# zdwww/EgoGaussian

Measured on AMD Instinct MI355X. Metric: train iters/s (fwd+bwd render) + PSNR, 500k Gaussians @ 960x540, higher is better.
Workload: dtype f32

## Files before the change

egogaussian_amd/csrc/api.hip:

```cpp
#include "egs_common.h"
#include "object_motion.h"
#include "backward_prologue.h"
#include "loss_window.h"
#include "label_bce.h"
#include "opacity_entropy.h"
#include <string.h>
#include <vector>
#include <mutex>
#include <unordered_map>
#include <stdlib.h>

namespace {

struct GeomLayout { egs_geom_layout o; size_t bytes; };
struct BinLayout { egs_binning_layout o; size_t bytes; };
struct ImgLayout { egs_image_layout o; size_t bytes; };

GeomLayout geom_layout(int P) {
    GeomLayout L; size_t off = 0; const size_t n = (size_t)(P > 0 ? P : 0);
    L.o.rec = off;          off = egs_align(off + n * sizeof(float4) * EGS_SPLAT_REC_F4);
    L.o.rect = off;         off = egs_align(off + n * sizeof(uint2));
    L.o.offsets = off;      off = egs_align(off + n * sizeof(uint32_t));
    L.o.clamped = off;      off = egs_align(off + n);
    L.o.visible = off;      off = egs_align(off + n);
// ... 498 lines not shown
        if (!entropy->weight || !entropy->n_vis || (P > 0 && !entropy->scratch) || c.obj_loss) return EGS_ERR_ARG;
        if (sc.act & EGS_ACT_OBJECT_MOTION) return EGS_ERR_MODE;
    }
    EgsObjRot orot; MotionHost mh; rc = obj_motion_args(sc, c.rot, orot, mh); if (rc) return rc;
    EgsLossGradHost lgh = {}; const EgsLossGradHost* lgp = nullptr; EgsObjLossK olk = {};
    if (c.obj_loss && !c.loss_grad) return EGS_ERR_ARG;
    if (c.loss_grad) {
        const egs_loss_grad& q = *c.loss_grad;
        if (!q.image || !q.gt || !q.dm_dmu1 || !q.dm_dexx || !q.dm_dexy || !q.upstream_grad) return EGS_ERR_ARG;
        if (c.dL_dout_depth || c.dL_dout_alpha || (c.grad_mask == EGS_GRAD_COLORS && sc.colors && !sink && !st.grad_accum)) return EGS_ERR_MODE;
        lgh = EgsLossGradHost{ q.image, q.gt, q.dm_dmu1, q.dm_dexx, q.dm_dexy, q.gate, q.upstream_grad, nullptr, 1.f - q.lambda_dssim, q.lambda_dssim,
                               q.deferred_partial_sums, q.deferred_partial_sums ? egs_l1_ssim_partial_count(3, height, width) / 2 : 0, q.lambda_dssim,
                               q.deferred_loss, q.deferred_partial_sums ? q.loss_running_sum : nullptr };
        lgp = &lgh;
        if (!dL_dout_color) dL_dout_color = q.image;
        if (c.obj_loss) {
            if (q.deferred_partial_sums && !c.obj_loss->alpha_partial_sums) return EGS_ERR_ARG;
            rc = obj_loss_args(c.obj_loss, 3, height, width, q.lambda_dssim, olk); if (rc) return rc;
            lgh.w_l1_n = c.obj_loss->lambda_image * (1.f - q.lambda_dssim); lgh.w_ssim_n = c.obj_loss->lambda_image * q.lambda_dssim;
            lgh.obj = &olk;
        }
    }
    if (P == 0) {
        if (lgp) EGS_TRY(egs_launch_loss_finish(lgh, width, height, s));
        if (entropy) EGS_TRY(egs_launch_entropy_reduce(0, nullptr, nullptr, 0, nullptr, nullptr, nullptr, nullptr, entropy->n_vis, entropy->value, s));
        if (mh.grad) EGS_TRY(egs_launch_zero_u32((uint32_t*)mh.grad, EGS_MOTION_SUMS, s));
        return 0;
    }
    if (R < 0 || R >= (1ll << 31)) return EGS_ERR_RANGE;
    if (c.grad_mask & ~EGS_GRAD_MASK_BITS) return EGS_ERR_ARG;
    const bool colors_only = c.grad_mask == EGS_GRAD_COLORS && sc.colors && !sink && !st.grad_accum;
    if (!c.background || lacks_pointers(sc, cam, c.radii, c.geom_buffer) || !c.image_buffer || !dL_dout_color || (!d.means2D && !colors_only) || !c.scratch)
        return EGS_ERR_ARG;
    if (misaligned(c.geom_buffer, c.binning_buffer, c.image_buffer) || ((uintptr_t)c.scratch & 15u)) return EGS_ERR_ARG;
    EgsGeomPtrs g = geom_ptrs(const_cast<void*>(c.geom_buffer), P);
    float* grad_acc = (float*)c.scratch;
    if (colors_only) {
        if (entropy) return EGS_ERR_MODE;
        if (!d.colors || (R > 0 && !c.binning_buffer)) return EGS_ERR_ARG;
        rc = check_modes(sc); if (rc) return rc;
        if (R == 0) return (int)egs_launch_zero_u32((uint32_t*)d.colors, (size_t)P * 3, s);
        EgsBinPtrs b = bin_ptrs(const_cast<void*>(c.binning_buffer), P, R, width, height);
        EgsImgPtrs im = img_ptrs(const_cast<void*>(c.image_buffer), width, height);
        if (!c.prologue_done) EGS_TRY(egs_launch_backward_prologue(P, width, height, im, grad_acc, g.block_hot, nullptr, s));
        void* det = nullptr; rc = det_lines_clear(c.scratch, P, debug, s, &det); if (rc) return rc;
        egs_prof_start(EGS_K_RENDER_BWD, s);
        EGS_TRY(egs_launch_render_backward(P, width, height, c.background, g, b.point_list, im, dL_dout_color, nullptr, nullptr, grad_acc, 1, nullptr, s, det));
        egs_prof_stop(EGS_K_RENDER_BWD, s);
        EGS_SYNC_IF_DEBUG(s);
        egs_prof_start(EGS_K_PREPROCESS_BWD, s);
        EGS_TRY(egs_launch_colors_from_acc(P, grad_acc, g.clamped, c.radii, d.colors, s));
        if (mh.grad) EGS_TRY(egs_launch_zero_u32((uint32_t*)mh.grad, EGS_MOTION_SUMS, s));
        egs_prof_stop(EGS_K_PREPROCESS_BWD, s);
        EGS_SYNC_IF_DEBUG(s);
        return 0;
    }
    const bool sh_apart = egs_sh_apart(sc);
    bool own[EGS_SINK_LEAVES] = { false, false, false, false, false, false };
    const bool sh_sink_ok = sh_apart && egs_sh_backward_can_sink(sc.M, sc.shs, sc.shs_rest);
    if (sink) {
        if (!sink->coef) return EGS_ERR_ARG;
        for (int l = 0; l < EGS_SINK_LEAVES; l++) {
            const egs_adam_leaf& f = sink->leaf[l];
            own[l] = f.param != nullptr;
            if (own[l] && (!f.exp_avg || !f.exp_avg_sq || !f.lr || !f.step)) return EGS_ERR_ARG;
        }
        if ((own[EGS_SINK_SCALES] || own[EGS_SINK_ROTATIONS]) && sc.cov3D) return EGS_ERR_MODE;
// ... 92 lines not shown
    return backward_impl({ BWD_SCENE, dL_dout_color, dL_dout_depth, dL_dout_alpha, BWD_OUTPUTS, BWD_SINK_TAIL, nullptr, nullptr, nullptr });
}

int egs_backward_lossgrad(int P, int sh_degree, int sh_coeffs, int64_t R, const float* background, const float* means3D,
                          const float* shs, const float* shs_rest, const float* colors_precomp, const float* scales, float scale_modifier,
                          const float* rotations, const float* cov3D_precomp, int activation_flags, const float* viewmatrix, const float* projmatrix,
                          const float* campos, int width, int height, float tan_fovx, float tan_fovy, const int32_t* radii,
                          const void* geom_buffer, const void* binning_buffer, const void* image_buffer, const egs_loss_grad* loss_grad,
                          float* dL_dmeans2D, float* dL_dcolors, float* dL_dopacity, float* dL_dmeans3D, float* dL_dcov3D, float* dL_dsh, float* dL_dsh_rest,
                          float* dL_dscales, float* dL_drotations, float* stat_grad_accum, float* stat_denom, float* stat_max_radii,
                          const uint32_t* skip_flag, const egs_adam_sink* sink, int prologue_done, const egs_object_rotation* rot, int grad_mask, void* scratch,
                          void* stream, int debug) {
    if (!loss_grad) return EGS_ERR_ARG;
    return backward_impl({ BWD_SCENE, nullptr, nullptr, nullptr, BWD_OUTPUTS, BWD_SINK_TAIL, loss_grad, nullptr, nullptr });
}

int egs_backward_entropy_lossgrad(int P, int sh_degree, int sh_coeffs, int64_t R, const float* background, const float* means3D,
                          const float* shs, const float* shs_rest, const float* colors_precomp, const float* scales, float scale_modifier,
                          const float* rotations, const float* cov3D_precomp, int activation_flags, const float* viewmatrix, const float* projmatrix,
                          const float* campos, int width, int height, float tan_fovx, float tan_fovy, const int32_t* radii,
                          const void* geom_buffer, const void* binning_buffer, const void* image_buffer, const egs_loss_grad* loss_grad,
                          const egs_opacity_entropy* entropy, const float* dL_dout_color, const float* dL_dout_depth, const float* dL_dout_alpha,
                          float* dL_dmeans2D, float* dL_dcolors, float* dL_dopacity, float* dL_dmeans3D, float* dL_dcov3D, float* dL_dsh, float* dL_dsh_rest,
                          float* dL_dscales, float* dL_drotations, float* stat_grad_accum, float* stat_denom, float* stat_max_radii,
                          const uint32_t* skip_flag, const egs_adam_sink* sink, int prologue_done, const egs_object_rotation* rot, int grad_mask, void* scratch,
                          void* stream, int debug) {
    if (!entropy) return EGS_ERR_ARG;
    if (loss_grad && (dL_dout_color || dL_dout_depth || dL_dout_alpha)) return EGS_ERR_MODE;
    return backward_impl({ BWD_SCENE, dL_dout_color, dL_dout_depth, dL_dout_alpha, BWD_OUTPUTS, BWD_SINK_TAIL, loss_grad, nullptr, entropy });
}

static int prologue_args(const egs_backward_prologue* side, EgsPrologueArgs& pa) {
    int rc = check_dims(side->P, side->width, side->height); if (rc) return rc;
    if (side->P <= 0 || !side->image_buffer || !side->scratch) return EGS_ERR_ARG;
    EgsImgPtrs im = img_ptrs(side->image_buffer, side->width, side->height);
    pa.n_tiles = (int)egs_tiles(side->width, side->height);
    pa.quad_work = im.quad_work; pa.tile_order = im.tile_order;
    if (side->geom_buffer && misaligned(side->geom_buffer)) return EGS_ERR_ARG;
    egs_prologue_acc(pa, (float*)side->scratch, (size_t)side->P,
                     side->geom_buffer ? geom_ptrs(const_cast<void*>(side->geom_buffer), side->P).block_hot : nullptr);
    if (side->sink) {
        if (!side->sink->coef) return EGS_ERR_ARG;
        EgsSink ks = {};
        sink_to_kernel_args(side->sink, side->skip_flag, ks, pa.tick);
        pa.has_tick = 1;
    }
    return 0;
}

int egs_l1_ssim_backward_ex(int channels, int height, int width, const float* img, const float* gt, float lambda_dssim,
                            const float* upstream_grad, const float* gate, const float* dm_dmu1, const float* dm_dexx,
                            const float* dm_dexy, float* dL_dimg, const float* deferred_partial_sums, float* deferred_loss,
                            float* loss_running_sum, const egs_backward_prologue* side, void* stream) {
    if (!side)
        return egs_launch_l1_ssim_backward(channels, height, width, img, gt, lambda_dssim, upstream_grad, gate, dm_dmu1, dm_dexx, dm_dexy, dL_dimg,
                                           deferred_partial_sums, deferred_loss, loss_running_sum, nullptr, (hipStream_t)stream);
    EgsPrologueArgs pa = {};
    int rc = prologue_args(side, pa); if (rc) return rc;
    return egs_launch_l1_ssim_backward(channels, height, width, img, gt, lambda_dssim, upstream_grad, gate, dm_dmu1, dm_dexx, dm_dexy, dL_dimg,
                                       deferred_partial_sums, deferred_loss, loss_running_sum, &pa, (hipStream_t)stream);
}

int egs_l1_ssim_forward_ex(int channels, int height, int width, const float* img, const float* gt, float lambda_dssim,
                           float* partial_sums, float* dm_dmu1, float* dm_dexx, float* dm_dexy, float* loss, float* loss_running_sum,
                           const egs_backward_prologue* side, void* stream) {
    EgsPrologueArgs pa = {};
    if (side) { int rc = prologue_args(side, pa); if (rc) return rc; }
// ... 62 lines not shown
}
int egs_label_bce_backward(int height, int width, const float* img, const float* obj_mask, const float* gate, const float* upstream_grad, float* dL_dimg,
                           const float* deferred_partial_sums, float* deferred_loss, float* loss_running_sum, void* stream) {
    int rc = check_dims(0, width, height); if (rc) return rc;
    if (!img || !obj_mask || !upstream_grad || !dL_dimg) return EGS_ERR_ARG;
    EGS_TRY(egs_launch_label_bce_backward(height, width, img, obj_mask, gate, upstream_grad, dL_dimg, deferred_partial_sums, deferred_loss,
                                          deferred_partial_sums ? loss_running_sum : nullptr, (hipStream_t)stream));
    return 0;
}
int egs_backward_label(int P, int64_t R, int width, int height, const int32_t* radii, const void* geom_buffer, const void* binning_buffer,
                       const void* image_buffer, const float* dL_dout_color, const egs_label_loss* loss, float* dL_dlabel, const egs_adam_leaf* adam,
                       float beta1, float beta2, float eps, float* coef, const int32_t* active_rows, const uint32_t* skip_flag, void* scratch,
                       void* stream, int flags) {
    const int debug = flags;
    int rc = check_dims(P, width, height); if (rc) return rc;
    if ((dL_dout_color != nullptr) == (loss != nullptr)) return EGS_ERR_MODE;
    if (R < 0 || R >= (1ll << 31)) return EGS_ERR_RANGE;
    const size_t n_partial = egs_label_bce_partial_count(height, width);
    if (loss && (!loss->img || !loss->mask || !loss->upstream || !loss->partial || loss->n_partial < n_partial)) return EGS_ERR_ARG;
    if (adam && (!adam->param || !adam->exp_avg || !adam->exp_avg_sq || !adam->lr || !adam->step || !coef)) return EGS_ERR_ARG;
    hipStream_t s = (hipStream_t)stream;
    const float inv_hw = 1.f / ((float)height * (float)width);
    EgsAdamTick tick = {}; EgsLabelAdam la = {};
    if (adam) {
        tick.step[0] = adam->step; tick.lr[0] = adam->lr; tick.coef = coef; tick.skip = skip_flag; tick.b1 = beta1; tick.b2 = beta2;
        la = EgsLabelAdam{ adam->param, adam->exp_avg, adam->exp_avg_sq, coef, active_rows, skip_flag, beta1, beta2, eps };
    }
    if (P == 0) {
        if (loss) EGS_TRY(egs_launch_label_bce_forward(height, width, loss->img, loss->mask, loss->partial, loss->loss, loss->running,
                                                       (loss->loss || loss->running) ? 1 : 0, s));
        return 0;
    }
    if (!radii || !geom_buffer || !image_buffer || !scratch || (R > 0 && !binning_buffer)) return EGS_ERR_ARG;
    if (misaligned(geom_buffer, binning_buffer, image_buffer) || ((uintptr_t)scratch & 15u)) return EGS_ERR_ARG;
    EgsGeomPtrs g = geom_ptrs(const_cast<void*>(geom_buffer), P);
    EgsImgPtrs im = img_ptrs(const_cast<void*>(image_buffer), width, height);
    float* grad_acc = (float*)scratch;
    if (R == 0) {
        EGS_TRY(egs_launch_zero_f4((float4*)grad_acc, egs_acc_floats((size_t)P) / 4, s));
        if (adam) EGS_TRY(egs_launch_adam_tick(tick, s));
        if (loss) EGS_TRY(egs_launch_label_bce_forward(height, width, loss->img, loss->mask, loss->partial, nullptr, nullptr, 0, s));
    } else {
        EgsBinPtrs b = bin_ptrs(const_cast<void*>(binning_buffer), P, R, width, height);
        EGS_TRY(egs_launch_backward_prologue(P, width, height, im, grad_acc, g.block_hot, adam ? &tick : nullptr, s));
        void* det = nullptr; rc = det_lines_clear(scratch, P, debug, s, &det); if (rc) return rc;
        EgsLabelLossK lk = {}; EgsLossGradHost lgh = {};
        if (loss) { lk = EgsLabelLossK{ loss->img, loss->mask, loss->gate, loss->upstream, loss->partial, inv_hw }; lgh.lab = &lk; }
        egs_prof_start(EGS_K_RENDER_BWD, s);
        EGS_TRY(egs_launch_render_backward(P, width, height, nullptr, g, b.point_list, im, dL_dout_color, nullptr, nullptr, grad_acc, 2, loss ? &lgh : nullptr, s, det));
        egs_prof_stop(EGS_K_RENDER_BWD, s);
        EGS_SYNC_IF_DEBUG(s);
    }
    egs_prof_start(EGS_K_PREPROCESS_BWD, s);
    EGS_TRY(egs_launch_label_finish(P, grad_acc, g.clamped, radii, dL_dlabel, adam ? &la : nullptr, skip_flag, loss ? loss->partial : nullptr, n_partial, inv_hw,
                                    loss ? loss->loss : nullptr, loss ? loss->running : nullptr, s));
    egs_prof_stop(EGS_K_PREPROCESS_BWD, s);
    EGS_SYNC_IF_DEBUG(s);
    return 0;
}

int egs_l1_ssim_pair_backward(int channels, int height, int width, const float* img, const float* gt, const float* upstream_l1,
                              const float* upstream_ssim, const float* gate, const float* dm_dmu1, const float* dm_dexx, const float* dm_dexy,
                              float* dL_dimg, const egs_backward_prologue* side, void* stream) {
    if (!upstream_l1 || !upstream_ssim) return EGS_ERR_ARG;
    EgsPrologueArgs pa = {};
    if (side) { int rc = prologue_args(side, pa); if (rc) return rc; }
    return egs_launch_l1_ssim_backward_w(channels, height, width, img, gt, 1.f, -1.f, 0.f, upstream_l1, upstream_ssim, gate, dm_dmu1, dm_dexx, dm_dexy, dL_dimg,
// ... 15 lines not shown
```

egogaussian_amd/csrc/egs_common.h:

```cpp
#pragma once
#include <hip/hip_runtime.h>
#include <stdint.h>
#include <stddef.h>
#include "../../include/egs_raster.h"

#define EGS_WAVE 64
#define EGS_SPLAT_REC_F4 3

#define EGS_LOG2E 1.4426950408889634f
#define EGS_LN2   0.6931471805599453f

#define EGS_GRAD_STRIDE 12

#ifndef EGS_HOT_MIN_TILES
#define EGS_HOT_MIN_TILES 256u
#endif
#define EGS_HOT_PER_BLOCK 7u
#define EGS_HOT_REPLICAS 8u
#define EGS_HOT_LINE 16u
#define EGS_BOX_MASK 0x7fffu
__host__ __device__ __forceinline__ uint32_t egs_hot_code(uint32_t bbx, uint32_t bby) {
    return ((bbx >> 15) & 1u) | ((bbx >> 30) & 2u) | ((bby >> 13) & 4u);
}
__host__ __device__ __forceinline__ void egs_hot_code_set(uint32_t& bbx, uint32_t& bby, uint32_t code) {
    bbx |= ((code & 1u) << 15) | ((code & 2u) << 30); bby |= (code & 4u) << 13;
}
__host__ __device__ static inline size_t egs_hot_slots(size_t P) { return ((P + 255) / 256) * EGS_HOT_PER_BLOCK; }
static inline size_t egs_hot_floats(size_t P) { return egs_hot_slots(P) * EGS_HOT_REPLICAS * EGS_HOT_LINE; }
static inline size_t egs_acc_floats(size_t P) { return P * EGS_GRAD_STRIDE + egs_hot_floats(P); }

struct EgsGeomPtrs {
    float4* rec; uint2* rect; uint32_t* offsets; uint8_t* clamped; uint8_t* visible; uint32_t* scan_scratch; uint64_t* total;
    uint32_t* block_hot;
};
#define EGS_CLAMP_MASK 7u
struct EgsBinPtrs {
    uint64_t* pairs;
    uint64_t* scratch;
    uint32_t* point_list;
    uint32_t* table;
    uint32_t* chunk_sum;
    uint32_t* flag;
    uint64_t* total;
    uint32_t* zero_after; uint32_t zero_after_n;
};
// ... 89 lines not shown
                                  EgsMotion mot, hipStream_t s);
bool egs_sh_backward_can_sink(int M, const float* sh_a, const float* sh_rest);
hipError_t egs_launch_mark_visible(int P, const float* means3D, const float* view, uint8_t* present, hipStream_t s);

hipError_t egs_launch_scan_u32(const uint32_t* in, uint32_t* out, size_t n, int inclusive, uint32_t* scratch,
                               uint64_t* total, hipStream_t s);
struct EgsSortArgs {
    int n_tiles; uint32_t stride; const uint32_t* table_scanned; const uint64_t* total; uint64_t* running_max; uint32_t* overflow_flag; int solo;
    uint32_t R ; int index_passes; uint64_t* pairs; uint64_t* scratch; uint32_t* point_list; uint2* ranges;
    uint32_t* zero_after; uint32_t zero_after_n; int rank_atomic ;
};
int egs_sort_plan(int P, int64_t R, int n_tiles, int call_flags );
hipError_t egs_launch_binning(int P, int64_t R, int W, int H, EgsGeomPtrs g, EgsBinPtrs b, EgsImgPtrs im,
                              uint64_t* running_max, uint32_t* overflow_flag, int sums_zeroed, int counted, EgsSortArgs* sort_in_blend, hipStream_t s, int call_flags );
bool egs_can_fuse_count(int P, int W, int H, int cull);
hipError_t egs_launch_preprocess_count(const EgsScene& sc, EgsCamera cam, int32_t* radii, EgsGeomPtrs g, EgsBinPtrs b,
                                       const int32_t* active_count, const EgsImgPtrs* place, EgsObjRot rot, EgsMotion mot, int cull, hipStream_t s);
hipError_t egs_launch_render_forward(int W, int H, const float* bg, EgsGeomPtrs g, const uint32_t* point_list,
                                     EgsImgPtrs im, float* out_color, float* out_depth, float* out_alpha, int placed,
                                     const EgsSortArgs* sort, hipStream_t s);
hipError_t egs_launch_backward_prologue(int P, int W, int H, EgsImgPtrs im, float* grad_acc, const uint32_t* block_hot, const EgsAdamTick* tick, hipStream_t s);
struct EgsLossGradHost { const float* img; const float* gt; const float* dm_dmu1; const float* dm_dexx; const float* dm_dexy; const float* gate;
                         const float* upstream; const float* upstream_ssim; float w_l1_n, w_ssim_n;
                         const float* fin_partial; size_t fin_n; float fin_lambda; float* fin_loss; float* fin_running;
                         const struct EgsObjLossK* obj; const struct EgsLabelLossK* lab; };
#ifdef EGS_LG_CHECK
extern EgsLossGradHost egs_debug_lossgrad;
#endif
hipError_t egs_launch_loss_finish(const EgsLossGradHost& lg, int W, int H, hipStream_t s);
hipError_t egs_launch_render_backward(int P, int W, int H, const float* bg, EgsGeomPtrs g, const uint32_t* point_list,
                                      EgsImgPtrs im, const float* dL_dcolor, const float* dL_ddepth,
                                      const float* dL_dalpha, float* grad_acc, int colors_only , const EgsLossGradHost* lg, hipStream_t s,
                                      void* det_lines = nullptr );
static inline size_t egs_det_bytes(size_t P) { return egs_align(P * EGS_GRAD_STRIDE * (sizeof(uint32_t) + sizeof(int64_t))); }
hipError_t egs_launch_colors_from_acc(int P, const float* grad_acc, const uint8_t* clamped, const int32_t* radii, float* dcolors, hipStream_t s);
struct EgsLabelAdam { float* p; float* m; float* v; const float* coef; const int32_t* active_rows; const uint32_t* skip; float b1, b2, eps; };
hipError_t egs_launch_label_finish(int P, const float* grad_acc, const uint8_t* clamped, const int32_t* radii, float* dlabel, const EgsLabelAdam* leaf,
                                   const uint32_t* skip, const float* partial, size_t n_partial, float inv_hw, float* loss, float* running, hipStream_t s);
hipError_t egs_launch_label_bce_forward(int H, int W, const float* img, const float* mask, float* partial, float* loss, float* running, int finish, hipStream_t s);
hipError_t egs_launch_label_bce_backward(int H, int W, const float* img, const float* mask, const float* gate, const float* up, float* dL_dimg,
                                         const float* fin_partial, float* fin_loss, float* fin_running, hipStream_t s);
hipError_t egs_launch_adam_tick(const EgsAdamTick& tick, hipStream_t s);

hipError_t egs_launch_zero_f4(float4* p, size_t n4, hipStream_t s);
hipError_t egs_launch_zero_u32(uint32_t* p, size_t n, hipStream_t s);

void egs_prof_start(int stage, hipStream_t s);
void egs_prof_stop(int stage, hipStream_t s);
```

egogaussian_amd/csrc/preprocess.hip:

```cpp
#include "egs_common.h"
#include <stdlib.h>
#include "bin_walk.h"
#include "backward_prologue.h"
#include "object_motion.h"
#include "opacity_entropy.h"
#include "sh_basis.h"
#include <type_traits>

namespace {

__device__ __forceinline__ void xform43(const float* p, const float* m, float* o) {
    o[0] = m[0] * p[0] + m[4] * p[1] + m[8] * p[2] + m[12];
    o[1] = m[1] * p[0] + m[5] * p[1] + m[9] * p[2] + m[13];
    o[2] = m[2] * p[0] + m[6] * p[1] + m[10] * p[2] + m[14];
}
__device__ __forceinline__ void xform44(const float* p, const float* m, float* o) {
    o[0] = m[0] * p[0] + m[4] * p[1] + m[8] * p[2] + m[12];
    o[1] = m[1] * p[0] + m[5] * p[1] + m[9] * p[2] + m[13];
    o[2] = m[2] * p[0] + m[6] * p[1] + m[10] * p[2] + m[14];
    o[3] = m[3] * p[0] + m[7] * p[1] + m[11] * p[2] + m[15];
}

__device__ __forceinline__ void quat_to_rot(const float* q, float* R) {
    float r = q[0], x = q[1], y = q[2], z = q[3];
// ... 271 lines not shown
                    egs_hot_code_set(bbx, bby, rank + 1u);
                    r2->z = __uint_as_float(bbx); r2->w = __uint_as_float(bby);
                    a.clamped_out[i] = (uint8_t)((a.clamped_out[i] & EGS_CLAMP_MASK) | ((rank + 1u) << 3));
                }
            }
        }
        bin_walk_round(L, bid, c.nblocks, g0, c.gpr, c.gx, false, c.cull != 0, c.use_map != 0, a.W, a.H,
                       [&](uint32_t tile, uint32_t, uint32_t) { atomicAdd(&hist[tile], 1u); });
        g0 += (unsigned)c.gpr;
    } while (!ONE_ROUND && g0 < per_block);
    __syncthreads();
    bin_flush_counts(hist, c.n_tiles, bid, c.stride, c.table, c.chunk_sum, blockIdx.x);
}

#define ST_MEANS 0
#define ST_OPAC 768
#define ST_SCALES 1024
#define ST_ROTS 1792
#define ST_SH 2816
template <bool SINK, int MOT, bool ENT = false>
__device__ __forceinline__ void pp_bwd_one(
    const int i, int D, int M, const float* __restrict__ means3D, const float* __restrict__ shs,
    const float* __restrict__ scales, float mod, const float* __restrict__ rots, const float* __restrict__ cov3D_in, int act,
    const float* __restrict__ V, const float* __restrict__ PM, const float* __restrict__ campos, int W, int H,
    float tanfovx, float tanfovy, const int32_t* __restrict__ radii, const uint8_t* __restrict__ clamped,
    const float4* __restrict__ rec, const float* __restrict__ grad_acc, const float* __restrict__ hot_acc, const size_t hot_slots, float* __restrict__ dmeans2D, float* __restrict__ dcolors,
    float* __restrict__ dopac, float* __restrict__ dmeans3D, float* __restrict__ dcov3D, float* __restrict__ dsh,
    float* __restrict__ dscales, float* __restrict__ drots,
    float* __restrict__ stat_grad_accum, float* __restrict__ stat_denom, float* __restrict__ stat_max_radii,
    const uint32_t* __restrict__ skip_flag, float* __restrict__ stage, const unsigned fused, const EgsObjRot rot, const EgsMotion mot, float* red,
    [[maybe_unused]] const float ent_coef = 0.f) {
    const unsigned tid = threadIdx.x;
    const bool vis = radii[i] > 0;
    float acc[EGS_GRAD_STRIDE];
    {
        const float4* ga = reinterpret_cast<const float4*>(grad_acc + (size_t)i * EGS_GRAD_STRIDE);
#pragma unroll
        for (int k = 0; k < 3; k++) {
            float4 v = vis ? ga[k] : make_float4(0.f, 0.f, 0.f, 0.f);
            acc[4 * k] = v.x; acc[4 * k + 1] = v.y; acc[4 * k + 2] = v.z; acc[4 * k + 3] = v.w;
        }
    }
    float gmx = 0.f, gmy = 0.f;
    if (vis) {
        const float4* r = rec + (size_t)i * EGS_SPLAT_REC_F4;
        const float4 r0 = r[0], r1 = r[1];
        const uint32_t code = (uint32_t)clamped[i] >> 3;
        if (code) {
            const float* hl = hot_acc + ((size_t)(i >> 8) * EGS_HOT_PER_BLOCK + (code - 1u)) * EGS_HOT_LINE;
            for (unsigned rp = 0; rp < EGS_HOT_REPLICAS; rp++) {
                const float4* ga = reinterpret_cast<const float4*>(hl + (size_t)rp * hot_slots * EGS_HOT_LINE);
#pragma unroll
                for (int k = 0; k < 3; k++) { const float4 v = ga[k]; acc[4 * k] += v.x; acc[4 * k + 1] += v.y; acc[4 * k + 2] += v.z; acc[4 * k + 3] += v.w; }
            }
        }
        const float cA = r0.z * (-2.f * EGS_LN2), cB = r0.w * (-EGS_LN2), cC = r1.x * (-2.f * EGS_LN2);
        const float o = r1.y;
        gmx = -o * (cA * acc[0] + cB * acc[1]); gmy = -o * (cC * acc[1] + cB * acc[0]);
        acc[2] *= -0.5f * o; acc[3] *= -0.5f * o; acc[4] *= -0.5f * o;
    }
    acc[0] = gmx * (0.5f * (float)W); acc[1] = gmy * (0.5f * (float)H);
    dmeans2D[3 * i] = acc[0]; dmeans2D[3 * i + 1] = acc[1]; dmeans2D[3 * i + 2] = 0.f;
    if (stat_grad_accum && vis && !(skip_flag && *skip_flag)) {
        stat_grad_accum[i] += sqrtf(acc[0] * acc[0] + acc[1] * acc[1]);
        stat_denom[i] += 1.f;
        if (stat_max_radii) stat_max_radii[i] = fmaxf(stat_max_radii[i], (float)radii[i]);
    }
// ... 404 lines not shown
```

egogaussian_amd/csrc/render_bwd.hip:

```cpp
#include "egs_common.h"
#include "blend_common.h"
#include "backward_prologue.h"
#include "blend_instrument.h"
#include "loss_window.h"
#include "label_bce.h"
#include "det_accum.h"
#include <algorithm>

namespace {

typedef unsigned uint2v __attribute__((ext_vector_type(2)));

__device__ __forceinline__ float fold32(float a, float b) {
    const uint2v r = __builtin_amdgcn_permlane32_swap(__float_as_uint(a), __float_as_uint(b), false, false);
    return __uint_as_float(r[0]) + __uint_as_float(r[1]);
}
__device__ __forceinline__ float fold16(float a, float b) {
    const uint2v r = __builtin_amdgcn_permlane16_swap(__float_as_uint(a), __float_as_uint(b), false, false);
    return __uint_as_float(r[0]) + __uint_as_float(r[1]);
}
template <int CTRL>
__device__ __forceinline__ float dpp_add(float v) {
    return v + __uint_as_float(__builtin_amdgcn_update_dpp(0u, __float_as_uint(v), CTRL, 0xf, 0xf, true));
}
__device__ __forceinline__ float row_sum(float v) {
    v = dpp_add<0xB1>(v);
    v = dpp_add<0x4E>(v);
    v = dpp_add<0x141>(v);
    v = dpp_add<0x140>(v);
    return v;
}
__device__ __forceinline__ float wave_sum_row3(float v) {
    v = row_sum(v);
    v += __uint_as_float(__builtin_amdgcn_update_dpp(0u, __float_as_uint(v), 0x142, 0xa, 0xf, false));
    v += __uint_as_float(__builtin_amdgcn_update_dpp(0u, __float_as_uint(v), 0x143, 0xc, 0xf, false));
    return v;
}

__global__ __launch_bounds__(1024) void k_backward_prologue(EgsPrologueArgs a) {
    __shared__ EgsOrderLds L;
    egs_prologue_job<1024>(a, blockIdx.x, gridDim.x, L);
}

#ifdef EGS_LG_CHECK
__device__ unsigned egs_lg_mismatch;
#endif
struct EgsLossGrad { const float* img; const float* gt; const float* m0; const float* m1; const float* m2; const float* gate;
                     const float* up; const float* up_ssim; float w_l1, w_ssim;
                     const float* fin_partial; size_t fin_n; float fin_lambda; float* fin_loss; float* fin_running;
                     EgsObjLossK obj; EgsLabelLossK lab; };
#define LG_COLS 27
template <int MODE, bool LG, int DET>
__global__ __launch_bounds__(256) __attribute__((amdgpu_waves_per_eu(8, 8))) void k_render_backward(
    int W, int H, int gx, int n_tiles, const uint2* __restrict__ ranges, const uint32_t* __restrict__ point_list,
    const float4* __restrict__ rec, const float* __restrict__ bg, const float* __restrict__ final_T,
    const uint32_t* __restrict__ n_contrib, const float* __restrict__ dL_dcolor, const float* __restrict__ dL_ddepth,
    const float* __restrict__ dL_dalpha, const uint32_t* __restrict__ tile_order, float* __restrict__ grad_acc,
    const uint32_t* __restrict__ quad_visits, const uint32_t hot_base ,
    const uint32_t hot_slots , const EgsLossGrad lg) {
    constexpr bool HAS_DA = MODE == 2;
    constexpr int NV = MODE == 0 ? 3 : MODE == 3 ? 1 : 10;
    constexpr bool COLOR_SUMS = MODE == 0 || MODE == 3;
    __shared__ float4 smem[4 * 64 * EGS_SPLAT_REC_F4 + 4 * 5 * 16];
    float4 (*lds)[64 * EGS_SPLAT_REC_F4] = reinterpret_cast<float4 (*)[64 * EGS_SPLAT_REC_F4]>(smem);
    float (*red)[5 * 64] = reinterpret_cast<float (*)[5 * 64]>(smem + 4 * 64 * EGS_SPLAT_REC_F4);
    static_assert(sizeof(smem) >= 9 * 16 * LG_COLS * sizeof(float), "the loss-gradient prologue's blurred maps fit the loop's LDS");
    __shared__ uint32_t quad_claimed;
    const uint32_t order_word = tile_order[blockIdx.x];
    if (order_word == 0xffffffffu) return;
    const int tile = (int)(order_word & ((order_word & EGS_ORDER_HAS_PERM) ? 0xffffu : 0xffffffffu));
    const unsigned lane = threadIdx.x & 63, wv = (unsigned)__builtin_amdgcn_readfirstlane((int)(threadIdx.x >> 6));
    unsigned q = wv;
    if (order_word & EGS_ORDER_HAS_PERM) {
        if (threadIdx.x == 0) quad_claimed = 0u;
        __syncthreads();
        uint32_t hw;
        asm volatile("s_getreg_b32 %0, hwreg(HW_REG_HW_ID)" : "=s"(hw));
        unsigned want = (order_word >> (16 + 2 * ((hw >> 4) & 3u))) & 3u;
        if (lane == 0) {
            uint32_t before = atomicOr(&quad_claimed, 1u << want);
            while (before & (1u << want)) {
                want = (unsigned)__builtin_ctz(~before & 0xfu);
                before = atomicOr(&quad_claimed, 1u << want);
            }
        }
        q = (unsigned)__builtin_amdgcn_readfirstlane((int)want);
    }
    float4* my = lds[wv];
    float* myred = red[wv];
    EGS_BWD_MEASURE(const uint64_t t_start = wall_clock64(); uint32_t meas = 0;)
    const int qx0 = (tile % gx) * EGS_TILE + (int)(q & 1) * 8, qy0 = (tile / gx) * EGS_TILE + (int)(q >> 1) * 8;
    const int px = qx0 + (int)(lane & 7), py = qy0 + (int)(lane >> 3);
    const bool inside = px < W && py < H;
    float lg_r = 0.f, lg_g = 0.f, lg_b = 0.f;
    if (LG && MODE != 3) {
        if (DET != 2 && lg.fin_partial && blockIdx.x == 0 && wv == 0) {
            if (HAS_DA) wave_finish_obj_loss(lg.fin_n, lg.fin_partial, lg.fin_lambda, lg.obj, lg.fin_loss, lg.fin_running, lane);
            else wave_finish_loss(lg.fin_n, lg.fin_partial, lg.w_l1, lg.w_ssim, lg.fin_lambda, lg.fin_loss, lg.fin_running, lane);
        }
        const int tx0 = (tile % gx) * EGS_TILE, ty0 = (tile / gx) * EGS_TILE;
        float* vb = reinterpret_cast<float*>(smem);
        const size_t HWp = (size_t)H * W;
        if (!(order_word & EGS_ORDER_HAS_PERM)) __syncthreads();
        if (threadIdx.x < 234) {
            const unsigned cm = threadIdx.x / 26u, col = threadIdx.x - cm * 26u, ch = cm / 3u, mp_i = cm - ch * 3u;
            const float* __restrict__ mp = (mp_i == 0 ? lg.m0 : mp_i == 1 ? lg.m1 : lg.m2) + ch * HWp;
            const int gxc = tx0 - 5 + (int)col;
            const bool colok = gxc >= 0 && gxc < W;
            float wv_[26];
#pragma unroll
            for (int r = 0; r < 26; r++) {
                const int gy_ = ty0 - 5 + r;
                const bool ok = colok && gy_ >= 0 && gy_ < H;
                wv_[r] = ok ? mp[(size_t)gy_ * W + gxc] : 0.f;
            }
            float* dst = vb + (size_t)cm * 16 * LG_COLS + col;
#pragma unroll
            for (int o = 0; o < 16; o++) {
                float acc = 0.f;
#pragma unroll
                for (int k = 0; k < 11; k++) acc = fmaf(kwin(k), wv_[o + k], acc);
// ... 50 lines not shown
    const uint32_t qx1 = (uint32_t)min(qx0 + 7, W - 1), qy1 = (uint32_t)min(qy0 + 7, H - 1);

    const uint2 range = ranges[tile];
    const uint32_t* list = point_list + range.x;

    float T_final = 0.f, g_r = 0.f, g_g = 0.f, g_b = 0.f, g_d = 0.f, g_a = 0.f;
    uint32_t last = 0;
    if (inside) {
        const size_t pix = (size_t)py * W + px, HW = (size_t)H * W;
        T_final = final_T[pix]; last = n_contrib[pix];
        if (MODE == 3) g_r = LG ? lg_r : __fadd_rn(__fadd_rn(dL_dcolor[pix], dL_dcolor[HW + pix]), dL_dcolor[2 * HW + pix]);
        else if (LG) { g_r = lg_r; g_g = lg_g; g_b = lg_b; }
        else { g_r = dL_dcolor[pix]; g_g = dL_dcolor[HW + pix]; g_b = dL_dcolor[2 * HW + pix]; }
#ifdef EGS_LG_CHECK
        if (LG && MODE != 3 && (__float_as_uint(lg_r) != __float_as_uint(dL_dcolor[pix]) || __float_as_uint(lg_g) != __float_as_uint(dL_dcolor[HW + pix]) ||
                   __float_as_uint(lg_b) != __float_as_uint(dL_dcolor[2 * HW + pix]))) atomicAdd(&egs_lg_mismatch, 1u);
#endif
        if (HAS_DA && !LG && dL_ddepth) g_d = dL_ddepth[pix];
        if (HAS_DA && !LG && dL_dalpha) g_a = dL_dalpha[pix];
        if (HAS_DA && LG) g_a = egs_alpha_grad(lg.obj.alpha[pix], lg.obj.mask[pix], lg.obj.w_l1a, lg.obj.w_l2a2, lg.up[0], lg.gate != nullptr,
                                               lg.gate ? lg.gate[pix] : 1.f);
    }
    const float bg_term = COLOR_SUMS ? 0.f : -T_final * (bg[0] * g_r + bg[1] * g_g + bg[2] * g_b);
    uint32_t wmax = last;
#pragma unroll
    for (int d = 32; d >= 1; d >>= 1) wmax = max(wmax, (uint32_t)__shfl_xor((int)wmax, d, 64));
    if (wmax == 0) return;
    if (MODE == 3 && __ballot(g_r != 0.f) == 0ull) return;

    const unsigned rv = lane >> 2, rg = lane & 3;
    const float4* red_src = reinterpret_cast<const float4*>(myred + (rv < (unsigned)NV ? (rv >> 1) * 64 + (rv & 1) * 32 + rg * 8 : 0));
    int slot = MODE == 3 ? (lane == 63 ? 6 : -1)
                         : (rg == 0 && rv < (unsigned)NV) ? (int)rv + (MODE == 0 ? 6 : 0) : -1;
    if (MODE == 3) asm volatile("" : "+v"(slot));

    float T = T_final, S = 0.f;
    EGS_BWD_ABL5(float abl_sink = 0.f;)

    EGS_LRPT(int remaining = (int)quad_visits[tile * 4 + q]; int prio_now = -1;)
    const int nb = (int)((wmax + 63) / 64);
    int b = nb - 1;
    uint32_t id_next = (uint32_t)b * 64 + lane < wmax ? list[(uint32_t)b * 64 + lane] : 0u;
    float4 r0, r1, r2;
    egs_load_rec(rec, id_next, (uint32_t)b * 64 + lane < wmax, r0, r1, r2);
    uint32_t id_cur = id_next;
    id_next = b >= 1 ? list[(uint32_t)(b - 1) * 64 + lane] : 0u;

    for (; b >= 0; b--) {
        const uint32_t base = (uint32_t)b * 64;
        const float4 c0 = r0, c1 = r1, c2 = r2;
        const uint32_t my_id = id_cur;
        const bool have = base + lane < wmax;
        egs_load_rec(rec, id_next, b >= 1, r0, r1, r2);
        id_cur = id_next;
        id_next = b >= 2 ? list[(uint32_t)(b - 2) * 64 + lane] : 0u;

        uint64_t mask = __ballot(have && egs_block_hits(c0, c1, c2, (uint32_t)qx0, qx1, (uint32_t)qy0, qy1));
        if (mask == 0ull) continue;
        my[lane * 3 + 0] = c0; my[lane * 3 + 1] = c1; my[lane * 3 + 2] = c2;
        __builtin_amdgcn_wave_barrier();
        const uint32_t my_code = egs_hot_code(__float_as_uint(c2.z), __float_as_uint(c2.w));
#ifdef EGS_NO_HOT
        const uint64_t hot_mask = 0ull; (void)my_code;
#else
        const uint64_t hot_mask = __ballot(have && my_code != 0u);
#endif
        const uint32_t lastb = last > base ? last - base : 0u;
        while (mask) {
            const int j = 63 - __builtin_clzll(mask);
            mask &= ~(1ull << j);
            EGS_LRPT({
                const int want = remaining >= 64 ? 3 : remaining >= 24 ? 2 : remaining >= 8 ? 1 : 0;
                if (want != prio_now) {
                    prio_now = want;
                    if (want == 3) __builtin_amdgcn_s_setprio(3); else if (want == 2) __builtin_amdgcn_s_setprio(2); else if (want == 1) __builtin_amdgcn_s_setprio(1); else __builtin_amdgcn_s_setprio(0);
                }
                remaining--;
            })
            const float4 s0 = my[j * 3 + 0], s1 = my[j * 3 + 1];
            const float2 s2 = *reinterpret_cast<const float2*>(&my[j * 3 + 2]);
            const float dx = s0.x - pxf, dy = s0.y - pyf;
            const float m = __fmul_rn(s0.z, dx);
            const float t = __fmaf_rn(s0.w, dy, m);
            const float nn = __fmul_rn(s1.x, dy);
            const float p = __fmaf_rn(nn, dy, __fmul_rn(t, dx));
            const float G = __builtin_amdgcn_exp2f(p);
            float a = fminf(0.99f, __fmul_rn(s1.y, G));
            a = p > 0.f ? 0.f : a;
            a = a < (1.0f / 255.0f) ? 0.f : a;
            a = ((uint32_t)j < lastb) ? a : 0.f;
            const bool contrib = a > 0.f;
            if (__ballot(contrib) == 0ull) continue;
            EGS_BWD_MEASURE(meas++;)
            const float rcp = __builtin_amdgcn_rcpf(1.f - a);
            const float Tn = T * rcp;
            const float w = a * Tn;
            float out;
            if (MODE == 3) {
                T = Tn;
                (void)S; (void)bg_term; (void)red_src; (void)myred;
                out = wave_sum_row3(w * g_r);
            } else {
            if (MODE == 0) {
                T = Tn;
                const float v6 = w * g_r, v7 = w * g_g, v8 = w * g_b;
                (void)S; (void)bg_term;
                myred[0 * 64 + lane] = fold32(v6, v7); myred[1 * 64 + lane] = fold32(v8, 0.f);
            } else {
            const float u = HAS_DA ? fmaf(s1.z, g_r, fmaf(s1.w, g_g, fmaf(s2.x, g_b, fmaf(s2.y, g_d, g_a))))
                                   : fmaf(s1.z, g_r, fmaf(s1.w, g_g, s2.x * g_b));
            float dLda = fmaf(bg_term, rcp, (u - S) * Tn);
            dLda = contrib ? dLda : 0.f;
            T = Tn; S = contrib ? fmaf(a, u - S, S) : S;

            const float gd = G * dLda;
            const float v0 = gd * dx, v1 = gd * dy;
            const float v2 = v0 * dx, v3 = v0 * dy, v4 = v1 * dy;
            const float v5 = gd;
            const float v6 = w * g_r, v7 = w * g_g, v8 = w * g_b, v9 = HAS_DA ? w * g_d : 0.f;

            EGS_BWD_ABL5(abl_sink += ((v0 + v1) + (v2 + v3)) + ((v4 + v5) + (v6 + v7)) + (v8 + v9); continue;)
            myred[0 * 64 + lane] = fold32(v0, v1); myred[1 * 64 + lane] = fold32(v2, v3); myred[2 * 64 + lane] = fold32(v4, v5);
            myred[3 * 64 + lane] = fold32(v6, v7); myred[4 * 64 + lane] = fold32(v8, v9);
            }
            const float4 pa = red_src[0], pb = red_src[1];
            out = ((pa.x + pa.y) + (pa.z + pa.w)) + ((pb.x + pb.y) + (pb.z + pb.w));
            out = dpp_add<0xB1>(out);
            out = dpp_add<0x4E>(out);
            }
            const uint32_t gid = (uint32_t)__builtin_amdgcn_readlane((int)my_id, j);
            if (DET != 0) {
                (void)hot_mask; (void)hot_slots;
                if (slot >= 0) {
                    uint32_t* det_max = reinterpret_cast<uint32_t*>(grad_acc);
                    const uint32_t word = gid * (uint32_t)EGS_GRAD_STRIDE + (uint32_t)slot;
                    if (DET == 1) atomicMax(det_max + word, egs_det_abs_bits(out));
                    else atomicAdd(reinterpret_cast<unsigned long long*>(det_max + hot_base) + word, (unsigned long long)egs_det_encode(out, det_max[word]));
                }
                continue;
            }
            EGS_BWD_ABL7(my[j * 3 + 2])
            uint32_t line = gid * (uint32_t)EGS_GRAD_STRIDE;
            if ((hot_mask >> j) & 1ull) {
                const uint32_t code = (uint32_t)__builtin_amdgcn_readlane((int)my_code, j);
                line = hot_base + ((blockIdx.x % EGS_HOT_REPLICAS) * hot_slots + (gid >> 8) * EGS_HOT_PER_BLOCK + code - 1u) * EGS_HOT_LINE;
            }
            if (slot >= 0) EGS_BWD_ACCUM(grad_acc + (line + (uint32_t)slot), out);
        }
        __builtin_amdgcn_wave_barrier();
    }
    EGS_BWD_ABL5(if (abl_sink == 12345.678f) grad_acc[lane] = abl_sink;)
    EGS_BWD_TIMELINE()
}

}

#ifdef EGS_LG_CHECK
EgsLossGradHost egs_debug_lossgrad = {};
#endif
namespace {
__global__ __launch_bounds__(64) void k_loss_finish(size_t n, const float* __restrict__ partial, float w_l1, float w_ssim, float lambda, float* loss, float* running) {
    wave_finish_loss(n, partial, w_l1, w_ssim, lambda, loss, running, threadIdx.x);
}
__global__ __launch_bounds__(64) void k_obj_loss_finish_wave(size_t n, const float* __restrict__ partial, float lambda, EgsObjLossK o, float* loss, float* running) {
    wave_finish_obj_loss(n, partial, lambda, o, loss, running, threadIdx.x);
}
}
hipError_t egs_launch_loss_finish(const EgsLossGradHost& lg, int W, int H, hipStream_t s) {
    if (!lg.fin_partial) return hipSuccess;
    const float n = (float)W * (float)H * 3.f;
    if (lg.obj) hipLaunchKernelGGL(k_obj_loss_finish_wave, dim3(1), dim3(64), 0, s, lg.fin_n, lg.fin_partial, lg.fin_lambda, *lg.obj, lg.fin_loss, lg.fin_running);
    else
    hipLaunchKernelGGL(k_loss_finish, dim3(1), dim3(64), 0, s, lg.fin_n, lg.fin_partial, lg.w_l1_n / n, lg.w_ssim_n / n, lg.fin_lambda, lg.fin_loss, lg.fin_running);
    return hipGetLastError();
}
#ifdef EGS_LG_CHECK
extern "C" unsigned egs_debug_lg_mismatches() { unsigned v = 0; (void)hipMemcpyFromSymbol(&v, HIP_SYMBOL(egs_lg_mismatch), sizeof(v)); return v; }
#endif
hipError_t egs_launch_backward_prologue(int P, int W, int H, EgsImgPtrs im, float* grad_acc, const uint32_t* block_hot, const EgsAdamTick* tick, hipStream_t s) {
    const int n_tiles = ((W + EGS_TILE - 1) / EGS_TILE) * ((H + EGS_TILE - 1) / EGS_TILE);
    if (n_tiles == 0) {
        if (tick) { hipError_t e = egs_launch_adam_tick(*tick, s); if (e != hipSuccess) return e; }
        return egs_launch_zero_f4((float4*)grad_acc, egs_acc_floats((size_t)P) / 4, s);
    }
    EgsPrologueArgs pa = {};
    pa.n_tiles = n_tiles; pa.quad_work = im.quad_work; pa.tile_order = im.tile_order;
    egs_prologue_acc(pa, grad_acc, (size_t)P, block_hot);
    pa.has_tick = tick ? 1 : 0; if (tick) pa.tick = *tick;
    hipLaunchKernelGGL(k_backward_prologue, dim3(egs_prologue_jobs(pa.n4, pa.has_tick, 1024)), dim3(1024), 0, s, pa);
    return hipGetLastError();
}

namespace {
__global__ __launch_bounds__(256) void k_det_decode(size_t n, const uint32_t* __restrict__ det_max, const int64_t* __restrict__ det_sum, float* __restrict__ grad_acc) {
    const size_t i = (size_t)blockIdx.x * 256 + threadIdx.x;
    if (i < n) grad_acc[i] = egs_det_decode(det_sum[i], det_max[i]);
}
}
hipError_t egs_launch_render_backward(int P, int W, int H, const float* bg, EgsGeomPtrs g, const uint32_t* point_list,
                                      EgsImgPtrs im, const float* dL_dcolor, const float* dL_ddepth,
                                      const float* dL_dalpha, float* grad_acc, int colors_only, const EgsLossGradHost* lg, hipStream_t s, void* det_lines) {
#ifdef EGS_LG_CHECK
    if (!lg && egs_debug_lossgrad.img) lg = &egs_debug_lossgrad;
#endif
    const int gx = (W + EGS_TILE - 1) / EGS_TILE, gy = (H + EGS_TILE - 1) / EGS_TILE;
    const int n_tiles = gx * gy;
    if (n_tiles == 0) return hipSuccess;
    EgsLossGrad lgk = {};
    if (lg) { lgk.img = lg->img; lgk.gt = lg->gt; lgk.m0 = lg->dm_dmu1; lgk.m1 = lg->dm_dexx; lgk.m2 = lg->dm_dexy; lgk.gate = lg->gate;
              lgk.up = lg->upstream; lgk.up_ssim = lg->upstream_ssim; lgk.w_l1 = lg->w_l1_n / ((float)W * (float)H * 3.f); lgk.w_ssim = lg->w_ssim_n / ((float)W * (float)H * 3.f);
              lgk.fin_partial = lg->fin_partial; lgk.fin_n = lg->fin_n; lgk.fin_lambda = lg->fin_lambda; lgk.fin_loss = lg->fin_loss; lgk.fin_running = lg->fin_running;
              if (lg->obj) lgk.obj = *lg->obj;
              if (lg->lab) lgk.lab = *lg->lab; }
#define EGS_BWD_LAUNCH_DET(MODE, LGF, DET, ACC) hipLaunchKernelGGL((k_render_backward<MODE, LGF, DET>), dim3(egs_blocks_for_tiles(n_tiles)), dim3(256), 0, s, W, H, gx, n_tiles, \
                           im.ranges, point_list, g.rec, bg, im.final_T, im.n_contrib, dL_dcolor, dL_ddepth, dL_dalpha, \
                           im.tile_order, ACC, im.quad_pairs + (size_t)4 * n_tiles, (uint32_t)((size_t)P * EGS_GRAD_STRIDE), (uint32_t)egs_hot_slots((size_t)P), lgk)
#define EGS_BWD_LAUNCH(MODE, LGF) do { if (!det_lines) EGS_BWD_LAUNCH_DET(MODE, LGF, 0, grad_acc); else { \
                           EGS_BWD_LAUNCH_DET(MODE, LGF, 1, (float*)det_lines); EGS_BWD_LAUNCH_DET(MODE, LGF, 2, (float*)det_lines); } } while (0)
    if (colors_only == 2 && lg && lg->lab) EGS_BWD_LAUNCH(3, true);
    else if (colors_only == 2) EGS_BWD_LAUNCH(3, false);
    else if (colors_only) EGS_BWD_LAUNCH(0, false);
    else if (lg && lg->obj) EGS_BWD_LAUNCH(2, true);
    else if (dL_ddepth || dL_dalpha) EGS_BWD_LAUNCH(2, false);
    else if (lg) EGS_BWD_LAUNCH(1, true);
    else EGS_BWD_LAUNCH(1, false);
    if (det_lines) {
        const size_t n = (size_t)P * EGS_GRAD_STRIDE;
        hipLaunchKernelGGL(k_det_decode, dim3((unsigned)((n + 255) / 256)), dim3(256), 0, s, n, (const uint32_t*)det_lines,
                           (const int64_t*)((const uint32_t*)det_lines + n), grad_acc);
    }
#undef EGS_BWD_LAUNCH_DET
#undef EGS_BWD_LAUNCH
    return hipGetLastError();
}

namespace {
__global__ __launch_bounds__(256) void k_colors_from_acc(int P, const float* __restrict__ grad_acc, const float* __restrict__ hot_acc, size_t hot_slots,
                                                         const uint8_t* __restrict__ clamped, const int32_t* __restrict__ radii,
                                                         float* __restrict__ dcolors) {
    const int i = blockIdx.x * 256 + threadIdx.x;
    if (i >= P) return;
    if (radii[i] <= 0) {
        dcolors[3 * (size_t)i] = 0.f; dcolors[3 * (size_t)i + 1] = 0.f; dcolors[3 * (size_t)i + 2] = 0.f;
        return;
    }
    const float4* ga = reinterpret_cast<const float4*>(grad_acc + (size_t)i * EGS_GRAD_STRIDE);
    const float4 a1 = ga[1], a2 = ga[2];
    float r = a1.z, g = a1.w, b = a2.x;
    const uint32_t code = (uint32_t)clamped[i] >> 3;
    if (code) {
        const float* hl = hot_acc + ((size_t)(i >> 8) * EGS_HOT_PER_BLOCK + (code - 1u)) * EGS_HOT_LINE;
        for (unsigned rp = 0; rp < EGS_HOT_REPLICAS; rp++) {
            const float4* h = reinterpret_cast<const float4*>(hl + (size_t)rp * hot_slots * EGS_HOT_LINE);
            const float4 h1 = h[1], h2 = h[2];
            r += h1.z; g += h1.w; b += h2.x;
        }
    }
    dcolors[3 * (size_t)i] = r; dcolors[3 * (size_t)i + 1] = g; dcolors[3 * (size_t)i + 2] = b;
}
}
// ... 7 lines not shown
```

Before: 3490.

## Pad gradient lines to 64 bytes and restructure backward LDS reduction rows

Widens the per-Gaussian gradient accumulator stride from 12 to 16 floats so each line fills a 64-byte aligned block, and tightens scratch alignment checks to match. The deterministic path keeps a separate 12-wide stride and remaps indices when decoding. The backward render kernel switches splat staging in LDS to a structure-of-arrays layout. For modes 1 and 2 it reduces through 8 unfolded rows written with ds_write_addtid inline assembly plus an extra DPP step, cutting fold work per splat. This costs more scratch memory and bandwidth per Gaussian and adds fragile inline asm tied to the M0 register.

```diff
diff --git a/egogaussian_amd/csrc/api.hip b/egogaussian_amd/csrc/api.hip
--- a/egogaussian_amd/csrc/api.hip
+++ b/egogaussian_amd/csrc/api.hip
@@ -554,7 +554,7 @@
     const bool colors_only = c.grad_mask == EGS_GRAD_COLORS && sc.colors && !sink && !st.grad_accum;
     if (!c.background || lacks_pointers(sc, cam, c.radii, c.geom_buffer) || !c.image_buffer || !dL_dout_color || (!d.means2D && !colors_only) || !c.scratch)
         return EGS_ERR_ARG;
-    if (misaligned(c.geom_buffer, c.binning_buffer, c.image_buffer) || ((uintptr_t)c.scratch & 15u)) return EGS_ERR_ARG;
+    if (misaligned(c.geom_buffer, c.binning_buffer, c.image_buffer) || ((uintptr_t)c.scratch & 63u)) return EGS_ERR_ARG;
     EgsGeomPtrs g = geom_ptrs(const_cast<void*>(c.geom_buffer), P);
     float* grad_acc = (float*)c.scratch;
     if (colors_only) {
@@ -713,7 +713,7 @@
 
 static int prologue_args(const egs_backward_prologue* side, EgsPrologueArgs& pa) {
     int rc = check_dims(side->P, side->width, side->height); if (rc) return rc;
-    if (side->P <= 0 || !side->image_buffer || !side->scratch) return EGS_ERR_ARG;
+    if (side->P <= 0 || !side->image_buffer || !side->scratch || ((uintptr_t)side->scratch & 63u)) return EGS_ERR_ARG;
     EgsImgPtrs im = img_ptrs(side->image_buffer, side->width, side->height);
     pa.n_tiles = (int)egs_tiles(side->width, side->height);
     pa.quad_work = im.quad_work; pa.tile_order = im.tile_order;
@@ -842,7 +842,7 @@
         return 0;
     }
     if (!radii || !geom_buffer || !image_buffer || !scratch || (R > 0 && !binning_buffer)) return EGS_ERR_ARG;
-    if (misaligned(geom_buffer, binning_buffer, image_buffer) || ((uintptr_t)scratch & 15u)) return EGS_ERR_ARG;
+    if (misaligned(geom_buffer, binning_buffer, image_buffer) || ((uintptr_t)scratch & 63u)) return EGS_ERR_ARG;
     EgsGeomPtrs g = geom_ptrs(const_cast<void*>(geom_buffer), P);
     EgsImgPtrs im = img_ptrs(const_cast<void*>(image_buffer), width, height);
     float* grad_acc = (float*)scratch;
diff --git a/egogaussian_amd/csrc/egs_common.h b/egogaussian_amd/csrc/egs_common.h
--- a/egogaussian_amd/csrc/egs_common.h
+++ b/egogaussian_amd/csrc/egs_common.h
@@ -10,7 +10,8 @@
 #define EGS_LOG2E 1.4426950408889634f
 #define EGS_LN2   0.6931471805599453f
 
-#define EGS_GRAD_STRIDE 12
+#define EGS_GRAD_STRIDE 16
+#define EGS_DET_STRIDE 12
 
 #ifndef EGS_HOT_MIN_TILES
 #define EGS_HOT_MIN_TILES 256u
@@ -166,7 +167,7 @@
                                       EgsImgPtrs im, const float* dL_dcolor, const float* dL_ddepth,
                                       const float* dL_dalpha, float* grad_acc, int colors_only , const EgsLossGradHost* lg, hipStream_t s,
                                       void* det_lines = nullptr );
-static inline size_t egs_det_bytes(size_t P) { return egs_align(P * EGS_GRAD_STRIDE * (sizeof(uint32_t) + sizeof(int64_t))); }
+static inline size_t egs_det_bytes(size_t P) { return egs_align(P * EGS_DET_STRIDE * (sizeof(uint32_t) + sizeof(int64_t))); }
 hipError_t egs_launch_colors_from_acc(int P, const float* grad_acc, const uint8_t* clamped, const int32_t* radii, float* dcolors, hipStream_t s);
 struct EgsLabelAdam { float* p; float* m; float* v; const float* coef; const int32_t* active_rows; const uint32_t* skip; float b1, b2, eps; };
 hipError_t egs_launch_label_finish(int P, const float* grad_acc, const uint8_t* clamped, const int32_t* radii, float* dlabel, const EgsLabelAdam* leaf,
diff --git a/egogaussian_amd/csrc/preprocess.hip b/egogaussian_amd/csrc/preprocess.hip
--- a/egogaussian_amd/csrc/preprocess.hip
+++ b/egogaussian_amd/csrc/preprocess.hip
@@ -327,7 +327,7 @@
     [[maybe_unused]] const float ent_coef = 0.f) {
     const unsigned tid = threadIdx.x;
     const bool vis = radii[i] > 0;
-    float acc[EGS_GRAD_STRIDE];
+    float acc[12];
     {
         const float4* ga = reinterpret_cast<const float4*>(grad_acc + (size_t)i * EGS_GRAD_STRIDE);
 #pragma unroll
diff --git a/egogaussian_amd/csrc/render_bwd.hip b/egogaussian_amd/csrc/render_bwd.hip
--- a/egogaussian_amd/csrc/render_bwd.hip
+++ b/egogaussian_amd/csrc/render_bwd.hip
@@ -50,6 +50,15 @@
                      const float* fin_partial; size_t fin_n; float fin_lambda; float* fin_loss; float* fin_running;
                      EgsObjLossK obj; EgsLabelLossK lab; };
 #define LG_COLS 27
+#define BWD_STAGE_F4 160
+#define BWD_RED_ROWS 8
+
+__device__ __forceinline__ void red_write_rows8(uint32_t slice_byte, float r0, float r1, float r2, float r3, float r4, float r5, float r6, float r7) {
+    asm volatile("s_mov_b32 m0, %8\n\ts_nop 1\n\t"
+                 "ds_write_addtid_b32 %0\n\tds_write_addtid_b32 %1 offset:256\n\tds_write_addtid_b32 %2 offset:512\n\tds_write_addtid_b32 %3 offset:768\n\t"
+                 "ds_write_addtid_b32 %4 offset:1024\n\tds_write_addtid_b32 %5 offset:1280\n\tds_write_addtid_b32 %6 offset:1536\n\tds_write_addtid_b32 %7 offset:1792"
+                 :: "v"(r0), "v"(r1), "v"(r2), "v"(r3), "v"(r4), "v"(r5), "v"(r6), "v"(r7), "s"(slice_byte) : "memory");
+}
 template <int MODE, bool LG, int DET>
 __global__ __launch_bounds__(256) __attribute__((amdgpu_waves_per_eu(8, 8))) void k_render_backward(
     int W, int H, int gx, int n_tiles, const uint2* __restrict__ ranges, const uint32_t* __restrict__ point_list,
@@ -61,9 +70,14 @@
     constexpr bool HAS_DA = MODE == 2;
     constexpr int NV = MODE == 0 ? 3 : MODE == 3 ? 1 : 10;
     constexpr bool COLOR_SUMS = MODE == 0 || MODE == 3;
-    __shared__ float4 smem[4 * 64 * EGS_SPLAT_REC_F4 + 4 * 5 * 16];
-    float4 (*lds)[64 * EGS_SPLAT_REC_F4] = reinterpret_cast<float4 (*)[64 * EGS_SPLAT_REC_F4]>(smem);
-    float (*red)[5 * 64] = reinterpret_cast<float (*)[5 * 64]>(smem + 4 * 64 * EGS_SPLAT_REC_F4);
+#ifdef EGS_RED5
+    constexpr bool ROWS8 = false;
+#else
+    constexpr bool ROWS8 = MODE == 1 || MODE == 2;
+#endif
+    __shared__ float4 smem[4 * BWD_STAGE_F4 + 4 * BWD_RED_ROWS * 16];
+    float4 (*lds)[BWD_STAGE_F4] = reinterpret_cast<float4 (*)[BWD_STAGE_F4]>(smem);
+    float (*red)[BWD_RED_ROWS * 64] = reinterpret_cast<float (*)[BWD_RED_ROWS * 64]>(smem + 4 * BWD_STAGE_F4);
     static_assert(sizeof(smem) >= 9 * 16 * LG_COLS * sizeof(float), "the loss-gradient prologue's blurred maps fit the loop's LDS");
     __shared__ uint32_t quad_claimed;
     const uint32_t order_word = tile_order[blockIdx.x];
@@ -87,6 +101,7 @@
         q = (unsigned)__builtin_amdgcn_readfirstlane((int)want);
     }
     float4* my = lds[wv];
+    float2* my_half = reinterpret_cast<float2*>(my + 128);
     float* myred = red[wv];
     EGS_BWD_MEASURE(const uint64_t t_start = wall_clock64(); uint32_t meas = 0;)
     const int qx0 = (tile % gx) * EGS_TILE + (int)(q & 1) * 8, qy0 = (tile / gx) * EGS_TILE + (int)(q >> 1) * 8;
@@ -203,6 +218,14 @@
     const float4* red_src = reinterpret_cast<const float4*>(myred + (rv < (unsigned)NV ? (rv >> 1) * 64 + (rv & 1) * 32 + rg * 8 : 0));
     int slot = MODE == 3 ? (lane == 63 ? 6 : -1)
                          : (rg == 0 && rv < (unsigned)NV) ? (int)rv + (MODE == 0 ? 6 : 0) : -1;
+    constexpr unsigned UNF = HAS_DA ? 6u : 7u;
+    const uint32_t red_byte = (uint32_t)__builtin_amdgcn_readfirstlane((int)(uint32_t)(uintptr_t)(__attribute__((address_space(3))) void*)myred);
+    const bool whole_row = lane < 8u * UNF;
+    if (ROWS8) {
+        red_src = reinterpret_cast<const float4*>(myred + 8 * lane);
+        slot = whole_row ? ((lane & 7u) == 0u ? (int)(lane >> 3) : -1) : ((lane & 3u) == 0u ? (int)(UNF + 2u * ((lane >> 3) - UNF) + ((lane >> 2) & 1u)) : -1);
+    }
+    const unsigned red_first = (lane >> 4) & 1u;
     if (MODE == 3) asm volatile("" : "+v"(slot));
 
     float T = T_final, S = 0.f;
@@ -228,7 +251,7 @@
 
         uint64_t mask = __ballot(have && egs_block_hits(c0, c1, c2, (uint32_t)qx0, qx1, (uint32_t)qy0, qy1));
         if (mask == 0ull) continue;
-        my[lane * 3 + 0] = c0; my[lane * 3 + 1] = c1; my[lane * 3 + 2] = c2;
+        my[lane] = c0; my[64 + lane] = c1; my_half[lane] = make_float2(c2.x, c2.y);
         __builtin_amdgcn_wave_barrier();
         const uint32_t my_code = egs_hot_code(__float_as_uint(c2.z), __float_as_uint(c2.w));
 #ifdef EGS_NO_HOT
@@ -248,8 +271,8 @@
                 }
                 remaining--;
             })
-            const float4 s0 = my[j * 3 + 0], s1 = my[j * 3 + 1];
-            const float2 s2 = *reinterpret_cast<const float2*>(&my[j * 3 + 2]);
+            const float4 s0 = my[j], s1 = my[64 + j];
+            const float2 s2 = my_half[j];
             const float dx = s0.x - pxf, dy = s0.y - pyf;
             const float m = __fmul_rn(s0.z, dx);
             const float t = __fmaf_rn(s0.w, dy, m);
@@ -291,26 +314,33 @@
             const float v6 = w * g_r, v7 = w * g_g, v8 = w * g_b, v9 = HAS_DA ? w * g_d : 0.f;
 
             EGS_BWD_ABL5(abl_sink += ((v0 + v1) + (v2 + v3)) + ((v4 + v5) + (v6 + v7)) + (v8 + v9); continue;)
+            if (ROWS8) {
+                if (HAS_DA) red_write_rows8(red_byte, v0, v1, v2, v3, v4, v5, fold32(v6, v7), fold32(v8, v9));
+                else red_write_rows8(red_byte, v0, v1, v2, v3, v4, v5, v6, fold32(v7, v8));
+            } else {
             myred[0 * 64 + lane] = fold32(v0, v1); myred[1 * 64 + lane] = fold32(v2, v3); myred[2 * 64 + lane] = fold32(v4, v5);
             myred[3 * 64 + lane] = fold32(v6, v7); myred[4 * 64 + lane] = fold32(v8, v9);
             }
-            const float4 pa = red_src[0], pb = red_src[1];
+            }
+            const float4 pa = red_src[ROWS8 ? red_first : 0u], pb = red_src[ROWS8 ? red_first ^ 1u : 1u];
             out = ((pa.x + pa.y) + (pa.z + pa.w)) + ((pb.x + pb.y) + (pb.z + pb.w));
             out = dpp_add<0xB1>(out);
             out = dpp_add<0x4E>(out);
+            if (ROWS8) { const float row = dpp_add<0x141>(out); out = whole_row ? row : out; }
             }
             const uint32_t gid = (uint32_t)__builtin_amdgcn_readlane((int)my_id, j);
             if (DET != 0) {
                 (void)hot_mask; (void)hot_slots;
                 if (slot >= 0) {
                     uint32_t* det_max = reinterpret_cast<uint32_t*>(grad_acc);
-                    const uint32_t word = gid * (uint32_t)EGS_GRAD_STRIDE + (uint32_t)slot;
+                    const uint32_t word = gid * (uint32_t)EGS_DET_STRIDE + (uint32_t)slot;
                     if (DET == 1) atomicMax(det_max + word, egs_det_abs_bits(out));
                     else atomicAdd(reinterpret_cast<unsigned long long*>(det_max + hot_base) + word, (unsigned long long)egs_det_encode(out, det_max[word]));
                 }
                 continue;
             }
-            EGS_BWD_ABL7(my[j * 3 + 2])
+            EGS_BWD_ABL7(make_float4(0.f, 0.f, __uint_as_float((uint32_t)__builtin_amdgcn_readlane((int)__float_as_uint(c2.z), j)),
+                                     __uint_as_float((uint32_t)__builtin_amdgcn_readlane((int)__float_as_uint(c2.w), j))))
             uint32_t line = gid * (uint32_t)EGS_GRAD_STRIDE;
             if ((hot_mask >> j) & 1ull) {
                 const uint32_t code = (uint32_t)__builtin_amdgcn_readlane((int)my_code, j);
@@ -365,7 +395,7 @@
 namespace {
 __global__ __launch_bounds__(256) void k_det_decode(size_t n, const uint32_t* __restrict__ det_max, const int64_t* __restrict__ det_sum, float* __restrict__ grad_acc) {
     const size_t i = (size_t)blockIdx.x * 256 + threadIdx.x;
-    if (i < n) grad_acc[i] = egs_det_decode(det_sum[i], det_max[i]);
+    if (i < n) { const size_t g = i / EGS_DET_STRIDE; grad_acc[g * EGS_GRAD_STRIDE + (i - g * EGS_DET_STRIDE)] = egs_det_decode(det_sum[i], det_max[i]); }
 }
 }
 hipError_t egs_launch_render_backward(int P, int W, int H, const float* bg, EgsGeomPtrs g, const uint32_t* point_list,
@@ -385,7 +415,7 @@
               if (lg->lab) lgk.lab = *lg->lab; }
 #define EGS_BWD_LAUNCH_DET(MODE, LGF, DET, ACC) hipLaunchKernelGGL((k_render_backward<MODE, LGF, DET>), dim3(egs_blocks_for_tiles(n_tiles)), dim3(256), 0, s, W, H, gx, n_tiles, \
                            im.ranges, point_list, g.rec, bg, im.final_T, im.n_contrib, dL_dcolor, dL_ddepth, dL_dalpha, \
-                           im.tile_order, ACC, im.quad_pairs + (size_t)4 * n_tiles, (uint32_t)((size_t)P * EGS_GRAD_STRIDE), (uint32_t)egs_hot_slots((size_t)P), lgk)
+                           im.tile_order, ACC, im.quad_pairs + (size_t)4 * n_tiles, (uint32_t)((size_t)P * ((DET) ? EGS_DET_STRIDE : EGS_GRAD_STRIDE)), (uint32_t)egs_hot_slots((size_t)P), lgk)
 #define EGS_BWD_LAUNCH(MODE, LGF) do { if (!det_lines) EGS_BWD_LAUNCH_DET(MODE, LGF, 0, grad_acc); else { \
                            EGS_BWD_LAUNCH_DET(MODE, LGF, 1, (float*)det_lines); EGS_BWD_LAUNCH_DET(MODE, LGF, 2, (float*)det_lines); } } while (0)
     if (colors_only == 2 && lg && lg->lab) EGS_BWD_LAUNCH(3, true);
@@ -396,7 +426,7 @@
     else if (lg) EGS_BWD_LAUNCH(1, true);
     else EGS_BWD_LAUNCH(1, false);
     if (det_lines) {
-        const size_t n = (size_t)P * EGS_GRAD_STRIDE;
+        const size_t n = (size_t)P * EGS_DET_STRIDE;
         hipLaunchKernelGGL(k_det_decode, dim3((unsigned)((n + 255) / 256)), dim3(256), 0, s, n, (const uint32_t*)det_lines,
                            (const int64_t*)((const uint32_t*)det_lines + n), grad_acc);
     }
```

Result: faster. 3612, median of 6 (+3.5%).
